# microsoft/DirectXTex

Hardware: AMD Instinct MI355X
Metric: Mtexels/s BC7 encode (4096^2 RGBA8, TEX_COMPRESS_DEFAULT) (higher is better)
Workload: dtype fp32 seed fit + i32 exact error sums (u8 texels in, 128-bit blocks out); 1 GPU; cfg2: 4096x4096 RGBA8 -> BC7_UNORM, TEX_COMPRESS_DEFAULT, one image per GPU, source and payload resident in HBM (dxtex_compress_device)

## Files before the change

### directxtex_amd/csrc/bc7_core.h

```cpp
#pragma once
#include <stdint.h>
#include <type_traits>

#if defined(DXTEX_HOST_DEBUG)
#define DXTEX_HD __host__ __device__ inline
#else
#define DXTEX_HD __device__ __forceinline__
#endif

namespace dxtex
{
namespace bc7
{
#if defined(DXTEX_HOST_DEBUG)
static bool g_hostFlatSkipEveryMode = true;
#endif
#if defined(DXTEX_COUNT_EVALS)
static long g_evalCount[8], g_evalTexels[8], g_macroCount[8], g_boundCount[8], g_pendCount[8], g_drainCount[8], g_pfTotal[8], g_pfPass[8], g_pfImprove[8], g_pfStepTotal[8][8], g_pfStepPass[8][8], g_tabWin[8], g_tabWinOut[8], g_tabWinOutPrev[8];
static int g_statTable = 0x7FFFFFFF, g_statTablePrev = 0x7FFFFFFF, g_statOther = 0;
static long g_rowCand[8], g_rowWin[8], g_rowTests[8][4], g_rowOut[8][4], g_rowDistN[8][6], g_rowDistOut[8][6], g_peelTests[8][4][3], g_peelOut[8][4][3];
#endif
template<int MODE> struct ModeInfo;
#define DXTEX_BC7_MODE(M, NS_, PARTBITS_, PB_, ROTBITS_, IMBITS_, IB_, IB2_, CP_, AP_, CPP_, APP_) \
    template<> struct ModeInfo<M> { enum : int { NS = NS_, PARTBITS = PARTBITS_, PB = PB_, ROTBITS = ROTBITS_, IMBITS = IMBITS_, \
// ... 1299 lines not shown
            ++g_pendCount[MODE];
#endif
        }
        exh_advance(s); --rem;
        const bool ended = rem == 0;
        if (n == 8 || ended)
        {
#if defined(DXTEX_COUNT_EVALS)
            if (n) ++g_drainCount[MODE];
#endif
            for (int j = n - 1; j >= 0; --j)
            {
                const uint32_t k = exh_key(exh_exact<MODE, IM, CHSET>(rg, vp, s.ch, s.aleb, s.o0, s.lo, queue[j], base), queue[j]);
                bestKey = k < bestKey ? k : bestKey;
            }
            n = 0;
        }
        if (ended)
        {
            exh_apply_key(s, bestKey);
            has = exh_next<MODE, IM, CHSET>(s, vp);
            skip_excluded();
            if (has) exh_peel<MODE, IM, CHSET>(rg, vp, s, base);
#if defined(DXTEX_ROW_STATS)
            row_stats(); peel_stats();
#endif
            if (has) { bestKey = exh_start_key(s); rem = exh_remaining(s); }
        }
    }
    optA = s.optA; optB = s.optB; optErr = s.optErr;
}

template<int MODE, int IM, class RG>
DXTEX_HD void optimize_one_lockstep(const RG& rg, int orgErr, uint32_t orgA, uint32_t orgB, uint32_t& optA, uint32_t& optB)
{
    optA = orgA; optB = orgB;
    int err = orgErr;
    if constexpr (PaletteBits<MODE, IM>::AB == 0)
    {
        lockstep_perturb_loop<MODE, IM, CH_ALL>(rg, optA, optB, err);
        lockstep_exhaustive_loop<MODE, IM, CH_ALL>(rg, optA, optB, err);
    }
    else
    {
        lockstep_perturb_loop<MODE, IM, CH_COLOR>(rg, optA, optB, err);
        lockstep_perturb_loop<MODE, IM, CH_ALPHA>(rg, optA, optB, err);
        lockstep_exhaustive_loop<MODE, IM, CH_COLOR>(rg, optA, optB, err);
        lockstep_exhaustive_loop<MODE, IM, CH_ALPHA>(rg, optA, optB, err);
    }
}

struct SubsetResult
{
    uint32_t orgA, orgB, optA, optB;
    uint64_t orgIdx1, orgIdx2, optIdx1, optIdx2;
    int orgErr, optErr;
};

template<int MODE, int IM, class RG>
DXTEX_HD void refine_pre(const RG& rg, uint32_t seedA, uint32_t seedB, uint32_t anchorPos, SubsetResult& out)
{
    const uint32_t qa = quantize_endpoint<MODE>(seedA), qb = quantize_endpoint<MODE>(seedB);
    fix_pbits<MODE>(qa, qb, out.orgA, out.orgB);
    out.orgErr = assign_indices<MODE, IM>(rg, out.orgA, out.orgB, anchorPos, out.orgIdx1, out.orgIdx2);
}

template<int MODE, int IM, class RG>
DXTEX_HD void refine_pre_err(const RG& rg, uint32_t seedA, uint32_t seedB, uint32_t anchorPos, SubsetResult& out)
{
    const uint32_t qa = quantize_endpoint<MODE>(seedA), qb = quantize_endpoint<MODE>(seedB);
    fix_pbits<MODE>(qa, qb, out.orgA, out.orgB);
    out.orgErr = assign_error<MODE, IM>(rg, out.orgA, out.orgB, anchorPos);
}

template<int MODE, int IM, class RG>
DXTEX_HD void refine_post(const RG& rg, uint32_t oa, uint32_t ob, uint32_t anchorPos, SubsetResult& out)
{
    fix_pbits<MODE>(oa, ob, out.optA, out.optB);
    out.optErr = assign_indices<MODE, IM>(rg, out.optA, out.optB, anchorPos, out.optIdx1, out.optIdx2);
}

template<int MODE, int IM, class RG>
DXTEX_HD void refine_subset(const RG& rg, uint32_t seedA, uint32_t seedB, uint32_t anchorPos, SubsetResult& out)
{
    refine_pre<MODE, IM>(rg, seedA, seedB, anchorPos, out);
    uint32_t oa, ob;
#if defined(DXTEX_BC7_USE_LOCKSTEP)
    optimize_one_lockstep<MODE, IM>(rg, out.orgErr, out.orgA, out.orgB, oa, ob);
#else
    optimize_one<MODE, IM>(rg, out.orgErr, out.orgA, out.orgB, oa, ob);
#endif
    refine_post<MODE, IM>(rg, oa, ob, anchorPos, out);
}

template<bool FULL, class F>
DXTEX_HD void for_masked(uint32_t mask16, F&& f)
{
    if constexpr (FULL)
    {
#pragma unroll
        for (int i = 0; i < 16; ++i) f(i);
    }
    else
    {
        for (uint32_t m = mask16 & 0xFFFFu; m; m &= m - 1u) f(int(__builtin_ctz(m)));
    }
}


template<bool RGBA, bool FULL = false, bool A1 = false>
DXTEX_HD bool fit_setup(const float* fpx, uint32_t mask16, float (&X)[4], float (&Y)[4])
{
// ... 456 lines not shown
```

### directxtex_amd/csrc/bc7_encode.hip

```cpp
#include "dxtex_kernels.h"
#include "bc67_tables.h"
#include "bc7_core.h"
#include "search_common.h"
#include <algorithm>
#include <cstdio>
#include <cstdlib>
#include <vector>

namespace dxtex
{
namespace
{
using namespace bc7;

struct Cand { uint32_t err; uint32_t ord; uint64_t lo, hi; };

enum : int { SLOT_M0 = 0, SLOT_M1, SLOT_M2, SLOT_M3, SLOT_M4A, SLOT_M4B, SLOT_M5, SLOT_M6, SLOT_M7, NUM_SLOTS };
enum : int { LIST_BYTES = 64 };

enum : int { PHASE_ALL = 0, PHASE_EARLY = 1, PHASE_LATE = 2 };

struct Bc7Args
{
    SegTable seg;
// ... 183 lines not shown
struct TaskRec { uint32_t A, B; int err; int orgErr; };

template<int MODE, int IM> struct TaskMap
{
    typedef ModeInfo<MODE> MI;
    enum : int { NS = MI::NS,
                 G = (NS == 1) ? 1 : (NS == 2) ? 2 : 4,
                 RANKS = (NS == 1) ? ((MODE == 6) ? 1 : 4) : ((MODE == 0) ? 4 : 16),
                 TPB = RANKS * G,
                 LIST = (MODE == 1) ? 0 : (MODE == 0) ? 33 : (MODE == 2) ? 40 : 16,
                 SLOT = (MODE == 0) ? SLOT_M0 : (MODE == 1) ? SLOT_M1 : (MODE == 2) ? SLOT_M2 : (MODE == 3) ? SLOT_M3 :
                        (MODE == 4) ? (IM ? SLOT_M4B : SLOT_M4A) : (MODE == 5) ? SLOT_M5 : (MODE == 6) ? SLOT_M6 : SLOT_M7 };
};

template<int MODE, int IM>
__device__ __forceinline__ uint32_t candidate_sub(uint32_t rank)
{
    return (TaskMap<MODE, IM>::NS == 1) ? ((MODE == 4) ? (rank * 2 + IM) * 16u : rank * 16u) : rank;
}
template<int MODE, int IM>
__device__ __forceinline__ uint32_t candidate_ord(uint32_t rank) { return uint32_t(MODE) * 128u + candidate_sub<MODE, IM>(rank); }

template<int MODE>
__device__ __forceinline__ bool phase_owns(const Bc7Args& a, uint32_t nb)
{
    if (a.phase == PHASE_ALL || (MODE != 4 && MODE != 5 && MODE != 6)) return true;
    const uint8_t* lst = a.lists + uint64_t(nb) * LIST_BYTES;
    const bool early = (MODE == 6) ? (lst[37] != 0 && a.flagged[0] >= a.early6Min) : (lst[32] != 0 && a.flagged[1] >= a.earlyAlphaMin);
    return early == (a.phase == PHASE_EARLY);
}

__device__ __forceinline__ bool lst_has_alpha(const Bc7Args& a, uint32_t nb) { return a.lists[uint64_t(nb) * LIST_BYTES + 32] != 0; }

template<int MODE, int IM>
__device__ __forceinline__ bool task_geometry(const Bc7Args& a, uint32_t nb, uint32_t r, uint32_t& shape, uint32_t& mask, uint32_t& anchor, uint32_t& rot)
{
    typedef TaskMap<MODE, IM> TM;
    shape = 0; mask = 0xFFFFu; anchor = 0; rot = 0;
    if (nb >= a.nblocks) return false;
    if (!phase_owns<MODE>(a, nb)) return false;
    const uint32_t rank = r / TM::G, region = r % TM::G;
    if (a.zeroOrd[nb] < candidate_ord<MODE, IM>(rank)) return false;
    if (TM::NS == 1) { rot = (MODE == 6) ? 0u : r; return true; }
    if (region >= uint32_t(TM::NS)) return false;
    const uint8_t* lst = a.lists + uint64_t(nb) * LIST_BYTES;
    if (MODE == 7 && lst[32] == 0) return false;
    shape = lst[TM::LIST + rank];
    if (TM::NS == 2)
    {
        const uint32_t m1 = kPart2Mask[shape];
        mask = region ? m1 : ((~m1) & 0xFFFFu);
        anchor = region ? uint32_t(kAnchor2[shape]) : 0u;
    }
    else
    {
        const uint32_t bits = kPart3Bits[shape];
        mask = 0;
#pragma unroll
        for (int i = 0; i < 16; ++i) if (((bits >> (2 * i)) & 3u) == region) mask |= 1u << i;
        anchor = (region == 0) ? 0u : (region == 1) ? uint32_t(kAnchor3[shape] & 15) : uint32_t(kAnchor3[shape] >> 4);
    }
    return true;
}

template<int MODE, int IM, bool ASSIGN = true>
__device__ __forceinline__ void task_org(const float* fpx, const uint32_t* pix, uint32_t mask, uint32_t anchor, uint32_t rot,
                                         SubsetResult& res, int& np, bool wantRegion, Region& rgOut, Block16& b16Out, const uint2* seed = nullptr)
{
    typedef TaskMap<MODE, IM> TM;
    if (TM::NS == 1)
    {
        block16_init(b16Out, pix, rot);
        uint32_t A, B;
        if (seed) { const uint2 sd = seed[(MODE == 6) ? 1 : 0]; A = sd.x; B = sd.y; }
        else if (MODE == 6) seed_endpoints<true>(fpx, 0xFFFFu, A, B);
// ... 24 lines not shown
    }
}

template<int BPW>
__device__ __forceinline__ void stage_packed(const Bc7Args& a, uint32_t nbFirst, int lane, uint32_t* sL)
{
    for (int t = lane; t < BPW * 16; t += 64)
    {
        const uint32_t nb = nbFirst + (uint32_t(t) >> 4);
        sL[t] = (nb < a.nblocks) ? a.px[uint64_t(nb) * 16 + (t & 15)] : 0u;
    }
    wave_lds_sync();
}

#if !defined(DXTEX_PP45_WGS)
#define DXTEX_PP45_WGS 1
#endif
template<int MODE, int IM>
__global__ void __launch_bounds__(256, (MODE == 4 || MODE == 5) ? DXTEX_PP45_WGS : 1) bc7_pre_kernel(Bc7Args a)
{
    typedef TaskMap<MODE, IM> TM;
    constexpr int BPW = (TM::TPB >= 64) ? 1 : 64 / TM::TPB;
    __shared__ uint32_t sL[4][BPW * 16];
    const int wave = threadIdx.x >> 6, lane = threadIdx.x & 63;
    const uint32_t nbFirst = (blockIdx.x * 4 + wave) * BPW;
    if (nbFirst >= a.nblocks) return;
    if (a.gate && *a.gate < a.gateMin) return;
    const uint32_t blk = uint32_t(lane) / TM::TPB, r = uint32_t(lane) % TM::TPB;
    const uint32_t nb = nbFirst + blk;
    uint32_t shape, mask, anchor, rot;
    const bool active = (blk < uint32_t(BPW)) && task_geometry<MODE, IM>(a, nb, r, shape, mask, anchor, rot);
    TaskRec rec; rec.A = 0; rec.B = 0; rec.err = 0; rec.orgErr = 0;
    uint32_t npLive = 0;
    if (!__any(active))
    {
        if (nb < a.nblocks && blk < uint32_t(BPW))
        {
            a.recs[uint64_t(nb) * TM::TPB + r] = rec;
            a.tinfo[uint64_t(nb) * TM::TPB + r] = 0;
        }
        return;
    }
    stage_packed<BPW>(a, nbFirst, lane, sL[wave]);
    int lb = 0;
    if (active)
    {
        SubsetResult res; int np; Region rg; Block16 b16;
        task_org<MODE, IM>(nullptr, &sL[wave][blk * 16], mask, anchor, rot, res, np, true, rg, b16,
                           (TM::NS == 2) ? a.seeds + uint64_t(nb) * 64 + (TM::LIST ? 32 : 0) + r
                                         : (TM::NS == 1) ? a.seeds1 + uint64_t(nb) * 2 : a.seeds3 + uint64_t(nb) * 192 + shape * 3 + (r % TM::G));
        rec.A = res.orgA; rec.B = res.orgB; rec.err = res.orgErr; rec.orgErr = res.orgErr;
        npLive = (res.orgErr != 0) ? uint32_t(np) : 0u;
        if (a.prune && npLive)
        {
            lb = subset_lower_bound(&sL[wave][blk * 16], mask, rot, (MODE >= 6) ? 4 : 3);
            if (MODE == 4 || MODE == 5)
            {
                if (rot != 0 || lst_has_alpha(a, nb))
                    lb += scalar_kmeans_lower_bound<(MODE == 4 && IM == 0) ? 8 : 4>(&sL[wave][blk * 16], rot);
            }
            if (MODE < 4)
            {
                const uint32_t* pix = &sL[wave][blk * 16];
#pragma unroll
                for (int i = 0; i < 16; ++i) if ((mask >> i) & 1u) { const int da = 255 - int(pix[i] >> 24); lb += da * da; }
            }
        }
    }
    if (a.prune)
    {
        int candOrg = active ? rec.err : 0, candLb = lb;
#pragma unroll
        for (int d = 1; d < TM::G; d <<= 1) { candOrg += __shfl_xor(candOrg, d); candLb += __shfl_xor(candLb, d); }
        int table = active ? candOrg : 0x7FFFFFFF;
#pragma unroll
        for (int d = TM::G; d < TM::TPB && d < 64; d <<= 1) table = min(table, __shfl_xor(table, d));
        if (nb < a.nblocks && blk < uint32_t(BPW)) table = min(table, a.bestErr[nb]);
        if (candLb > table) npLive = 0;
    }
    if (nb < a.nblocks && blk < uint32_t(BPW))
    {
        a.recs[uint64_t(nb) * TM::TPB + r] = rec;
        a.tinfo[uint64_t(nb) * TM::TPB + r] = (mask & 0xFFFFu) | (rot << 16) | (npLive << 24);
    }
}

template<int MODE, int IM>
__device__ __forceinline__ void search_pickup(const Bc7Args& a, uint2 task, uint32_t* slotCol, SlotRegion& rg)
{
    typedef TaskMap<MODE, IM> TM;
    const uint32_t nb = task.x / TM::TPB;
    const uint32_t mask = task.y & 0xFFFFu, rot = (task.y >> 16) & 3u;
    const uint4* px4 = reinterpret_cast<const uint4*>(a.px + uint64_t(nb) * 16);
    const uint4 q0 = px4[0], q1 = px4[1], q2 = px4[2], q3 = px4[3];
    const uint32_t px[16] = { q0.x, q0.y, q0.z, q0.w, q1.x, q1.y, q1.z, q1.w, q2.x, q2.y, q2.z, q2.w, q3.x, q3.y, q3.z, q3.w };
    int np = 0;
    if (TM::NS == 1)
    {
#pragma unroll
        for (int i = 0; i < 16; ++i) slotCol[i * kSlotStride] = rotate_pixel(px[i], rot);
        np = 16;
    }
    else
    {
#pragma unroll
        for (int i = 0; i < 16; ++i)
            if ((mask >> i) & 1u) { slotCol[np * kSlotStride] = px[i]; ++np; }
    }
    rg.base = slotCol; rg.np = np; rg.p2sum = 0;
}

__device__ __forceinline__ int lanes_below(unsigned long long mask)
{
    return int(__builtin_amdgcn_mbcnt_hi(uint32_t(mask >> 32), __builtin_amdgcn_mbcnt_lo(uint32_t(mask), 0u)));
}

// ... 671 lines not shown
                const int o = oStart + c / 11, i = st.lo + c % 11;
                const bool valid = c < 121 && o < st.oEnd && i < st.iEnd && i >= o;
                int e = 0x7FFFFFFF;
                if (valid)
                {
                    const int av = st.aleb ? o : i, bv = st.aleb ? i : o;
                    e = eval_var<MODE, IM, CHSET>(rg, vp, ch, unq1<C::PREC>(uint32_t(av)), unq1<C::PREC>(uint32_t(bv)), base);
                }
                const uint64_t key = valid ? ((uint64_t(uint32_t(e)) << 8) | uint32_t(c)) : ~0ull;
                bestKey = key < bestKey ? key : bestKey;
            }
#pragma unroll
            for (int d = 32; d > 0; d >>= 1)
            {
                const uint32_t lo = uint32_t(__shfl_xor(int(uint32_t(bestKey)), d)), hi = uint32_t(__shfl_xor(int(uint32_t(bestKey >> 32)), d));
                const uint64_t other = (uint64_t(hi) << 32) | lo;
                bestKey = other < bestKey ? other : bestKey;
            }
            if (bestKey != ~0ull)
            {
                const int e = int(uint32_t(bestKey >> 8)), c = int(bestKey & 0xFFu);
                if (e < st.best) { st.best = e; st.omin = oStart + c / 11; st.imin = st.lo + c % 11; }
            }
            st = exh_commit(st);
        }
        if (lane == 0)
        {
            TaskRec* r = a.recs + task.x;
            r->A = st.optA; r->B = st.optB; r->err = st.optErr;
        }
    }
}

template<int MODE, int IM>
__global__ void __launch_bounds__(256, (MODE == 4 || MODE == 5) ? DXTEX_PP45_WGS : 1) bc7_post_kernel(Bc7Args a)
{
    typedef TaskMap<MODE, IM> TM;
    constexpr int BPW = (TM::TPB >= 64) ? 1 : 64 / TM::TPB;
    __shared__ uint32_t sL[4][BPW * 16];
    const int wave = threadIdx.x >> 6, lane = threadIdx.x & 63;
    const uint32_t nbFirst = (blockIdx.x * 4 + wave) * BPW;
    if (nbFirst >= a.nblocks) return;
    if (a.gate && *a.gate < a.gateMin) return;
    const uint32_t blk = uint32_t(lane) / TM::TPB, r = uint32_t(lane) % TM::TPB;
    const uint32_t nb = nbFirst + blk;
    const uint32_t rank = r / TM::G, region = r % TM::G;
    uint32_t shape, mask, anchor, rot;
    const bool active = (blk < uint32_t(BPW)) && task_geometry<MODE, IM>(a, nb, r, shape, mask, anchor, rot);
    const bool mine = blk < uint32_t(BPW) && nb < a.nblocks && phase_owns<MODE>(a, nb);
    if (!__any(active))
    {
        if (mine && r == 0)
        {
            Cand c; c.err = 0xFFFFFFFFu; c.ord = 0xFFFFFFFFu; c.lo = 0; c.hi = 0;
            a.cands[uint64_t(nb) * NUM_SLOTS + TM::SLOT] = c;
        }
        return;
    }
    stage_packed<BPW>(a, nbFirst, lane, sL[wave]);

    SubsetResult res;
    res.orgErr = 0; res.optErr = 0; res.orgA = res.orgB = res.optA = res.optB = 0;
    res.orgIdx1 = res.orgIdx2 = res.optIdx1 = res.optIdx2 = 0;
    int np = 0; Region rg; Block16 b16;
    if (active)
    {
        task_org<MODE, IM, false>(nullptr, &sL[wave][blk * 16], mask, anchor, rot, res, np, true, rg, b16,
                                  (TM::NS == 2) ? a.seeds + uint64_t(nb) * 64 + (TM::LIST ? 32 : 0) + r
// ... 28 lines not shown
    uint64_t idx1 = myIdx1;
#pragma unroll
    for (int s = 1; s < TM::NS; ++s)
    {
        epA[s] = uint32_t(__shfl_down(int(myA), s));
        epB[s] = uint32_t(__shfl_down(int(myB), s));
        const uint64_t oi = uint64_t(uint32_t(__shfl_down(int(uint32_t(myIdx1)), s))) |
                            (uint64_t(uint32_t(__shfl_down(int(uint32_t(myIdx1 >> 32)), s))) << 32);
        idx1 |= oi;
    }

    if (blk < uint32_t(BPW) && nb < a.nblocks && region == 0)
    {
        if (active && key == best)
        {
            uint32_t anchors[3] = { 0, 0, 0 };
            if (TM::NS == 2) anchors[1] = kAnchor2[shape];
            if (TM::NS == 3) { anchors[1] = kAnchor3[shape] & 15; anchors[2] = kAnchor3[shape] >> 4; }
            Cand c;
            c.err = uint32_t(err);
            c.ord = uint32_t(MODE) * 128u + sub;
            emit_block<MODE>(shape, rot, IM, epA, epB, idx1, myIdx2, anchors, c.lo, c.hi);
            a.cands[uint64_t(nb) * NUM_SLOTS + TM::SLOT] = c;
            if (err == 0) atomicMin(&a.zeroOrd[nb], c.ord);
            atomicMin(&a.bestErr[nb], err);
        }
        else if (!active && rank == 0 && mine)
        {
            Cand c; c.err = 0xFFFFFFFFu; c.ord = 0xFFFFFFFFu; c.lo = 0; c.hi = 0;
            a.cands[uint64_t(nb) * NUM_SLOTS + TM::SLOT] = c;
        }
    }
}

template<bool RGBA>
__global__ void __launch_bounds__(256) bc7_block_seeds_kernel(Bc7Args a)
{
    const uint32_t nb = blockIdx.x * 256u + threadIdx.x;
    if (nb >= a.nblocks) return;
    const BcSeg& sg = seg_of(a.seg, nb);
    float f[64];
#pragma unroll
    for (int t = 0; t < 16; ++t) { uint32_t ldr; load_block_texel(sg.src, sg.nbw, sg.nb0 + (nb - sg.l0), uint32_t(t), &f[t * 4], ldr); }
    uint32_t A, B;
    seed_endpoints<RGBA, true>(f, 0xFFFFu, A, B);
    a.seeds1[uint64_t(nb) * 2 + (RGBA ? 1 : 0)] = make_uint2(A, B);
}

__global__ void __launch_bounds__(256) bc7_flag_count_kernel(Bc7Args a, uint32_t* out)
{
    uint32_t n = 0, m = 0;
    for (uint32_t nb = blockIdx.x * 256u + threadIdx.x; nb < a.nblocks; nb += gridDim.x * 256u)
    {
        uint8_t* lst = a.lists + uint64_t(nb) * LIST_BYTES;
        const bool hasAlpha = lst[32] != 0;
        bool first = hasAlpha;
        if (!first)
        {
            const uint4* px4 = reinterpret_cast<const uint4*>(a.px + uint64_t(nb) * 16);
            const uint4 q0 = px4[0], q1 = px4[1], q2 = px4[2], q3 = px4[3];
            const uint32_t px[16] = { q0.x, q0.y, q0.z, q0.w, q1.x, q1.y, q1.z, q1.w, q2.x, q2.y, q2.z, q2.w, q3.x, q3.y, q3.z, q3.w };
            const int ea = *reinterpret_cast<const int*>(lst + 56);
            first = int64_t(subset_lower_bound(px, 0xFFFFu, 0u, 4)) * 100 <= int64_t(ea) * a.early6Pct;
        }
        lst[37] = first ? 1 : 0;
        n += first ? 1u : 0u;
// ... 49 lines not shown
struct ScratchLayout
{
    size_t lists, cands, px, recs, order, tinfo, counters, zeroOrd, bestErr, seeds, seeds1, seeds3, flagcnt, auxRecs, auxOrder, auxTinfo, auxCounters, total;
    size_t auxTpb, auxSlices;
    explicit ScratchLayout(uint64_t nb, bool threeSubsets)
    {
        auto up = [](size_t v) { return (v + 255) & ~size_t(255); };
        const size_t tpb = threeSubsets ? kMaxTasksPerBlock : 32;
        const bool small = nb <= kSmallPassBlocks;
        auxTpb = small ? tpb : 4; auxSlices = small ? size_t(kSideStreams) : 2;
        size_t o = 0;
        lists = o; o = up(o + nb * LIST_BYTES);
        cands = o; o = up(o + nb * NUM_SLOTS * sizeof(Cand));
        px = o; o = up(o + nb * 64);
        recs = o; o = up(o + nb * tpb * sizeof(TaskRec));
        order = o; o = up(o + nb * tpb * sizeof(uint2));
        tinfo = o; o = up(o + nb * tpb * sizeof(uint32_t));
        counters = o; o = up(o + 64 * sizeof(uint32_t));
        zeroOrd = o; o = up(o + nb * sizeof(uint32_t));
        bestErr = o; o = up(o + nb * sizeof(int));
        seeds = o; o = up(o + nb * 64 * sizeof(uint2));
        seeds1 = o; o = up(o + nb * 2 * sizeof(uint2));
        seeds3 = o; o = up(o + (threeSubsets ? nb * 192 * sizeof(uint2) : 0));
        flagcnt = o; o = up(o + 256);
        auxRecs = o; o = up(o + auxSlices * nb * auxTpb * sizeof(TaskRec));
        auxOrder = o; o = up(o + auxSlices * nb * auxTpb * sizeof(uint2));
        auxTinfo = o; o = up(o + auxSlices * nb * auxTpb * sizeof(uint32_t));
        auxCounters = o; o = up(o + size_t(kSideStreams) * 64 * sizeof(uint32_t));
        total = o;
    }
};

template<int MODE, int IM>
void launch_mode(const Bc7Args& a0, hipStream_t stream, KernelMarks* marks, const char* const (&names)[7])
{
    typedef TaskMap<MODE, IM> TM;
    constexpr int BPW = (TM::TPB >= 64) ? 1 : 64 / TM::TPB;
    const uint32_t nb = a0.nblocks;
    const uint32_t ntasks = nb * uint32_t(TM::TPB);
    const uint32_t gridPP = (nb + 4 * BPW - 1) / (4 * BPW);
    constexpr bool kWhole = TM::NS == 1;
    constexpr uint32_t kExhMax = (MODE == 6) ? kWaveTaskMax : kWaveTaskMax45;
    static const bool noGroup = dev_env("DXTEX_BC7_NO_GROUP") != nullptr;
    const bool maybeShortP = kWhole && !noGroup && (MODE == 6 || ntasks <= 4u * kPerturbWaveMax);
    const bool maybeShortE = kWhole && !noGroup && (MODE == 6 || ntasks <= 4u * kExhMax);
    const uint32_t wavesP = std::min<uint32_t>(kSearchWaves, (ntasks + 1) / 2), wavesE = std::min<uint32_t>(kSearchWaves, ntasks);
    Bc7Args a = a0;
    a.gate = nullptr; a.gateMin = 0;
    if (a0.flagged && !(a0.flags & BCF_BC7_QUICK))
    {
        if (MODE == 7) { a.gate = a0.flagged + 1; a.gateMin = 1; }
        else if (a0.phase == PHASE_EARLY && (MODE == 4 || MODE == 5)) { a.gate = a0.flagged + 1; a.gateMin = std::max<uint32_t>(1u, a0.earlyAlphaMin); }
        else if (a0.phase == PHASE_EARLY && MODE == 6) { a.gate = a0.flagged; a.gateMin = std::max<uint32_t>(1u, a0.early6Min); }
    }
    a.perturbWaveMax = maybeShortP ? kPerturbWaveMax : 0u;
    a.exhWaveMax = maybeShortE ? kExhMax : 0u;
    if (marks) marks->mark(names[0]);
    hipLaunchKernelGGL((bc7_pre_kernel<MODE, IM>), dim3(gridPP), dim3(256), 0, stream, a);
    if (marks) marks->mark(names[1]);
    (void)hipMemsetAsync(a.counters, 0, 64 * sizeof(uint32_t), stream);
    const uint32_t binGroups = std::min<uint32_t>(kBinGroups, (ntasks + 255) / 256);
    hipLaunchKernelGGL(bc7_bin_count_kernel, dim3(binGroups), dim3(256), 0, stream, a.tinfo, ntasks, a.counters, a.gate, a.gateMin);
    hipLaunchKernelGGL(bc7_bin_scan_kernel, dim3(1), dim3(1), 0, stream, a.counters);
    hipLaunchKernelGGL(bc7_bin_scatter_kernel, dim3(binGroups), dim3(256), 0, stream, a.tinfo, ntasks, a.counters, a.order, a.gate, a.gateMin);
    if (marks) marks->mark(names[2]);
    const uint32_t waves = std::min<uint32_t>(kSearchWaves, (ntasks + 63) / 64);
    static const int tailBelow = dev_env("DXTEX_BC7_TAIL_BELOW") ? atoi(dev_env("DXTEX_BC7_TAIL_BELOW")) : 48;
// ... 5 lines not shown
        if constexpr (MODE == 1 || MODE == 6)
        {
            if (perturbPlain) hipLaunchKernelGGL((bc7_perturb_kernel<MODE, IM, CH_ALL>), dim3(waves), dim3(64), 0, stream, a, 0);
            else hipLaunchKernelGGL((bc7_perturb_filter_kernel<MODE, IM, CH_ALL>), dim3(waves), dim3(64), 0, stream, a, 0);
        }
        else
            hipLaunchKernelGGL((bc7_perturb_kernel<MODE, IM, CH_ALL>), dim3(waves), dim3(64), 0, stream, a, 0);
        if constexpr (kWhole) { if (maybeShortP) hipLaunchKernelGGL((bc7_perturb_wave_kernel<MODE, IM, CH_ALL>), dim3(wavesP), dim3(64), 0, stream, a); }
        if (marks) marks->mark(names[4]);
        if constexpr (kWhole) { if (maybeShortE) hipLaunchKernelGGL((bc7_exhaustive_wave_kernel<MODE, IM, CH_ALL>), dim3(wavesE), dim3(64), 0, stream, a); }
        hipLaunchKernelGGL((bc7_exhaustive_kernel<MODE, IM, CH_ALL>), dim3(waves), dim3(64), 0, stream, a, 1, tailBelow, rangeTests);
    }
    else
    {
        if constexpr (MODE == 4 && IM == 1 && DXTEX_PF_M4 != 0)
        {
            if (perturbPlain) hipLaunchKernelGGL((bc7_perturb_kernel<MODE, IM, CH_COLOR>), dim3(waves), dim3(64), 0, stream, a, 0);
            else hipLaunchKernelGGL((bc7_perturb_filter_kernel<MODE, IM, CH_COLOR>), dim3(waves), dim3(64), 0, stream, a, 0);
        }
        else
            hipLaunchKernelGGL((bc7_perturb_kernel<MODE, IM, CH_COLOR>), dim3(waves), dim3(64), 0, stream, a, 0);
        if (maybeShortP) hipLaunchKernelGGL((bc7_perturb_wave_kernel<MODE, IM, CH_COLOR>), dim3(wavesP), dim3(64), 0, stream, a);
        if (marks) marks->mark(names[3]);
        hipLaunchKernelGGL((bc7_perturb_kernel<MODE, IM, CH_ALPHA>), dim3(waves), dim3(64), 0, stream, a, 1);
        if (maybeShortP) hipLaunchKernelGGL((bc7_perturb_wave_kernel<MODE, IM, CH_ALPHA>), dim3(wavesP), dim3(64), 0, stream, a);
        if (marks) marks->mark(names[4]);
        if (maybeShortE) hipLaunchKernelGGL((bc7_exhaustive_wave_kernel<MODE, IM, CH_COLOR>), dim3(wavesE), dim3(64), 0, stream, a);
        hipLaunchKernelGGL((bc7_exhaustive_kernel<MODE, IM, CH_COLOR>), dim3(waves), dim3(64), 0, stream, a, 2, tailBelow, rangeTests);
        if (marks) marks->mark(names[5]);
        if (maybeShortE) hipLaunchKernelGGL((bc7_exhaustive_wave_kernel<MODE, IM, CH_ALPHA>), dim3(wavesE), dim3(64), 0, stream, a);
        hipLaunchKernelGGL((bc7_exhaustive_kernel<MODE, IM, CH_ALPHA>), dim3(waves), dim3(64), 0, stream, a, 3, tailBelow, rangeTests);
    }
    if (marks) marks->mark(names[6]);
    hipLaunchKernelGGL((bc7_post_kernel<MODE, IM>), dim3(gridPP), dim3(256), 0, stream, a);
#if defined(DXTEX_DEV)
    static const bool stats = dev_env("DXTEX_BC7_STATS") != nullptr;
    if (stats)
    {
        uint32_t c[40] = {};
        (void)hipStreamSynchronize(stream);
        (void)hipMemcpy(c, a.counters, sizeof(c), hipMemcpyDeviceToHost);
        std::fprintf(stderr, "bc7 stats %-22s phase %d: %9u task slots, %9u live; by size 16..1:", names[0], a.phase, ntasks, c[34]);
        for (int b = 16; b >= 1; --b) std::fprintf(stderr, " %u", c[b]);
        std::fprintf(stderr, "\n");
    }
#endif
}
}

#if defined(DXTEX_BC7_WAVETIMES)
namespace
{
void bc7_wavetimes_report()
{
    (void)hipDeviceSynchronize();
    static int call = 0;
    static const int wanted = dev_env("DXTEX_BC7_WT_CALL") ? atoi(dev_env("DXTEX_BC7_WT_CALL")) : 2;
    const bool print = call++ == wanted;
    static std::vector<unsigned long long> h(size_t(WT_KEYS) * 8192 * WT_FIELDS);
    static std::vector<unsigned int> hist(size_t(WT_KEYS) * 256);
    (void)hipMemcpyFromSymbol(h.data(), HIP_SYMBOL(g_wt), h.size() * 8);
    (void)hipMemcpyFromSymbol(hist.data(), HIP_SYMBOL(g_wtHist), hist.size() * 4);
    unsigned long long tAll = ~0ull;
    for (size_t i = 0; i < size_t(WT_KEYS) * 8192; ++i) if (h[i * WT_FIELDS + 2]) tAll = std::min(tAll, h[i * WT_FIELDS]);
    static const char* const kinds[3] = { "perturb", "perturb_filter", "exhaustive" };
    for (int key = 0; key < WT_KEYS; ++key)
    {
// ... 32 lines not shown
        }
        {
            const unsigned long long* e = w + idx[idx.size() / 2] * WT_FIELDS;
            std::fprintf(stderr, "    median wavefront %d: start %.0f drained %.0f end %.0f %% of span, rounds %llu, busy lanes / round %.1f, tasks %llu\n", idx[idx.size() / 2],
                         100.0 * double(e[0] - t0) / dur, 100.0 * double(e[1] - t0) / dur, 100.0 * double(e[2] - t0) / dur, e[3], e[3] ? double(e[4]) / e[3] : 0.0, e[5]);
        }
    }
    std::fill(h.begin(), h.end(), 0ull); std::fill(hist.begin(), hist.end(), 0u);
    (void)hipMemcpyToSymbol(HIP_SYMBOL(g_wt), h.data(), h.size() * 8);
    (void)hipMemcpyToSymbol(HIP_SYMBOL(g_wtHist), hist.data(), hist.size() * 4);
}
}
#endif

size_t bc7_scratch_bytes(uint64_t nblocks, uint32_t flags, size_t nimages)
{
    const bool three = (flags & BCF_USE_3SUBSETS) != 0;
    size_t need = ScratchLayout(nblocks < kMaxBlocksPerPass ? nblocks : kMaxBlocksPerPass, three).total;
    if (nblocks > kSmallPassBlocks) need = std::max(need, ScratchLayout(kSmallPassBlocks, three).total);
    return need + seg_table_bytes(nblocks, kMaxBlocksPerPass, nimages);
}

hipError_t launch_bc7_encode(const SrcView& src, uint8_t* dst, uint64_t dstRowPitch, uint32_t flags,
                             void* scratch, hipStream_t stream, KernelMarks* marks, const SideStreams* side)
{
    BcImage one; one.src = src; one.dst = dst; one.dstRowPitch = dstRowPitch;
    return launch_bc7_encode_many(&one, 1, flags, scratch, stream, marks, side);
}

hipError_t launch_bc7_encode_many(const BcImage* images, size_t count, uint32_t flags, void* scratch, hipStream_t stream, KernelMarks* marks,
                                  const SideStreams* side)
{
#define DXTEX_MARK(NAME) do { if (marks) marks->mark(NAME); } while (0)
#define DXTEX_MODE(MODE, IM, TAG) do { static const char* const n_[7] = { "bc7_pre_" TAG, "bc7_bin_" TAG, "bc7_perturb_" TAG, "bc7_perturb_alpha_" TAG, \
                                           "bc7_exhaustive_" TAG, "bc7_exhaustive_alpha_" TAG, "bc7_post_" TAG }; \
                                       launch_mode<MODE, IM>(a, stream, marks, n_); } while (0)
    std::vector<BcSeg> segs;
    std::vector<BcPass> passes;
    uint64_t perPass = 0;
    if (!build_passes(images, count, kMaxBlocksPerPass, segs, passes, &perPass)) return hipSuccess;
    const bool three = (flags & BCF_USE_3SUBSETS) != 0;
    const ScratchLayout L(perPass, three);
    uint8_t* base = static_cast<uint8_t*>(scratch);
    BcSeg* dSegs = reinterpret_cast<BcSeg*>(base + L.total);
    const hipError_t ce = upload_segments(dSegs, segs, passes, stream);
    if (ce != hipSuccess) return ce;
    const bool quick = (flags & BCF_BC7_QUICK) != 0;

    for (const BcPass& pass : passes)
    {
        Bc7Args a;
        set_pass(a.seg, dSegs, segs, pass);
        a.nblocks = pass.nblocks;
        a.flags = flags;
        a.perturbWaveMax = 0; a.exhWaveMax = 0;
        a.gate = nullptr; a.gateMin = 0;
        a.lists = base + L.lists;
        a.cands = reinterpret_cast<Cand*>(base + L.cands);
        a.px = reinterpret_cast<uint32_t*>(base + L.px);
        a.recs = reinterpret_cast<TaskRec*>(base + L.recs);
        a.order = reinterpret_cast<uint2*>(base + L.order);
        a.tinfo = reinterpret_cast<uint32_t*>(base + L.tinfo);
        a.counters = reinterpret_cast<uint32_t*>(base + L.counters);
        a.zeroOrd = reinterpret_cast<uint32_t*>(base + L.zeroOrd);
        a.bestErr = reinterpret_cast<int*>(base + L.bestErr);
        a.seeds = reinterpret_cast<uint2*>(base + L.seeds);
        a.seeds1 = reinterpret_cast<uint2*>(base + L.seeds1);
        a.seeds3 = reinterpret_cast<uint2*>(base + L.seeds3);
// ... 154 lines not shown
```

Before: 136.6 Mtexels/s.

## Split BC7 post into error-only selection and winner-only emit kernel

Result: no change. 137.7 Mtexels/s, median of 6 (+0.8%).

```diff
diff --git a/directxtex_amd/csrc/bc7_core.h b/directxtex_amd/csrc/bc7_core.h
--- a/directxtex_amd/csrc/bc7_core.h
+++ b/directxtex_amd/csrc/bc7_core.h
@@ -1355,7 +1355,7 @@
 }
 
 template<int MODE, int IM, class RG>
-DXTEX_HD void optimize_one_lockstep(const RG& rg, int orgErr, uint32_t orgA, uint32_t orgB, uint32_t& optA, uint32_t& optB)
+DXTEX_HD void optimize_one_lockstep(const RG& rg, int orgErr, uint32_t orgA, uint32_t orgB, uint32_t& optA, uint32_t& optB, int* errOut = nullptr)
 {
     optA = orgA; optB = orgB;
     int err = orgErr;
@@ -1371,6 +1371,7 @@
         lockstep_exhaustive_loop<MODE, IM, CH_COLOR>(rg, optA, optB, err);
         lockstep_exhaustive_loop<MODE, IM, CH_ALPHA>(rg, optA, optB, err);
     }
+    if (errOut) *errOut = err;
 }
 
 struct SubsetResult
@@ -1401,6 +1402,13 @@
 {
     fix_pbits<MODE>(oa, ob, out.optA, out.optB);
     out.optErr = assign_indices<MODE, IM>(rg, out.optA, out.optB, anchorPos, out.optIdx1, out.optIdx2);
+}
+
+template<int MODE, int IM, class RG>
+DXTEX_HD void refine_post_err(const RG& rg, uint32_t oa, uint32_t ob, uint32_t anchorPos, SubsetResult& out)
+{
+    fix_pbits<MODE>(oa, ob, out.optA, out.optB);
+    out.optErr = assign_error<MODE, IM>(rg, out.optA, out.optB, anchorPos);
 }
 
 template<int MODE, int IM, class RG>
diff --git a/directxtex_amd/csrc/bc7_encode.hip b/directxtex_amd/csrc/bc7_encode.hip
--- a/directxtex_amd/csrc/bc7_encode.hip
+++ b/directxtex_amd/csrc/bc7_encode.hip
@@ -239,15 +239,17 @@
 
 __device__ __forceinline__ bool lst_has_alpha(const Bc7Args& a, uint32_t nb) { return a.lists[uint64_t(nb) * LIST_BYTES + 32] != 0; }
 
-template<int MODE, int IM>
+constexpr uint32_t kTaskPruned = 1u << 23;
+
+template<int MODE, int IM, bool LIVE = true>
 __device__ __forceinline__ bool task_geometry(const Bc7Args& a, uint32_t nb, uint32_t r, uint32_t& shape, uint32_t& mask, uint32_t& anchor, uint32_t& rot)
 {
     typedef TaskMap<MODE, IM> TM;
     shape = 0; mask = 0xFFFFu; anchor = 0; rot = 0;
     if (nb >= a.nblocks) return false;
-    if (!phase_owns<MODE>(a, nb)) return false;
+    if (LIVE && !phase_owns<MODE>(a, nb)) return false;
     const uint32_t rank = r / TM::G, region = r % TM::G;
-    if (a.zeroOrd[nb] < candidate_ord<MODE, IM>(rank)) return false;
+    if (LIVE && a.zeroOrd[nb] < candidate_ord<MODE, IM>(rank)) return false;
     if (TM::NS == 1) { rot = (MODE == 6) ? 0u : r; return true; }
     if (region >= uint32_t(TM::NS)) return false;
     const uint8_t* lst = a.lists + uint64_t(nb) * LIST_BYTES;
@@ -338,6 +340,7 @@
     const bool active = (blk < uint32_t(BPW)) && task_geometry<MODE, IM>(a, nb, r, shape, mask, anchor, rot);
     TaskRec rec; rec.A = 0; rec.B = 0; rec.err = 0; rec.orgErr = 0;
     uint32_t npLive = 0;
+    uint32_t pruned = 0;
     if (!__any(active))
     {
         if (nb < a.nblocks && blk < uint32_t(BPW))
@@ -382,12 +385,12 @@
 #pragma unroll
         for (int d = TM::G; d < TM::TPB && d < 64; d <<= 1) table = min(table, __shfl_xor(table, d));
         if (nb < a.nblocks && blk < uint32_t(BPW)) table = min(table, a.bestErr[nb]);
-        if (candLb > table) npLive = 0;
+        if (candLb > table) { npLive = 0; pruned = kTaskPruned; }
     }
     if (nb < a.nblocks && blk < uint32_t(BPW))
     {
         a.recs[uint64_t(nb) * TM::TPB + r] = rec;
-        a.tinfo[uint64_t(nb) * TM::TPB + r] = (mask & 0xFFFFu) | (rot << 16) | (npLive << 24);
+        a.tinfo[uint64_t(nb) * TM::TPB + r] = (mask & 0xFFFFu) | (rot << 16) | pruned | (npLive << 24);
     }
 }
 
@@ -1125,8 +1128,157 @@
     }
 }
 
+constexpr uint32_t kParkedOpt = 1u << 31;
+
 template<int MODE, int IM>
 __global__ void __launch_bounds__(256, (MODE == 4 || MODE == 5) ? DXTEX_PP45_WGS : 1) bc7_post_kernel(Bc7Args a)
+{
+    typedef TaskMap<MODE, IM> TM;
+    constexpr int BPW = (TM::TPB >= 64) ? 1 : 64 / TM::TPB;
+    __shared__ uint32_t sL[4][BPW * 16];
+    const int wave = threadIdx.x >> 6, lane = threadIdx.x & 63;
+    const uint32_t nbFirst = (blockIdx.x * 4 + wave) * BPW;
+    if (nbFirst >= a.nblocks) return;
+    if (a.gate && *a.gate < a.gateMin) return;
+    const uint32_t blk = uint32_t(lane) / TM::TPB, r = uint32_t(lane) % TM::TPB;
+    const uint32_t nb = nbFirst + blk;
+    const uint32_t rank = r / TM::G, region = r % TM::G;
+    uint32_t shape, mask, anchor, rot;
+    bool active = (blk < uint32_t(BPW)) && task_geometry<MODE, IM>(a, nb, r, shape, mask, anchor, rot);
+    const bool mine = blk < uint32_t(BPW) && nb < a.nblocks && phase_owns<MODE>(a, nb);
+    if (active && (a.tinfo[uint64_t(nb) * TM::TPB + r] & kTaskPruned)) active = false;
+    if (!__any(active))
+    {
+        if (mine && r == 0)
+        {
+            Cand c; c.err = 0xFFFFFFFFu; c.ord = 0xFFFFFFFFu; c.lo = 0; c.hi = 0;
+            a.cands[uint64_t(nb) * NUM_SLOTS + TM::SLOT] = c;
+        }
+        return;
+    }
+    stage_packed<BPW>(a, nbFirst, lane, sL[wave]);
+
+    SubsetResult res;
+    res.orgErr = 0; res.optErr = 0; res.optA = res.optB = 0;
+    if (active)
+    {
+        const TaskRec rec = a.recs[uint64_t(nb) * TM::TPB + r];
+        res.orgErr = rec.orgErr;
+        if (TM::NS == 1)
+        {
+            Block16 b16; block16_init(b16, &sL[wave][blk * 16], rot);
+            refine_post_err<MODE, IM>(b16, rec.A, rec.B, 0u, res);
+        }
+        else
+        {
+            Region rg; region_init(rg, &sL[wave][blk * 16], mask);
+            refine_post_err<MODE, IM>(rg, rec.A, rec.B, anchor, res);
+        }
+    }
+    int orgTot = res.orgErr, optTot = res.optErr;
+#pragma unroll
+    for (int d = 1; d < TM::G; d <<= 1) { orgTot += __shfl_xor(orgTot, d); optTot += __shfl_xor(optTot, d); }
+    const bool useOpt = optTot < orgTot;
+    const int err = useOpt ? optTot : orgTot;
+    const uint32_t sub = candidate_sub<MODE, IM>(rank);
+    const uint32_t key = active ? ((uint32_t(err) << 7) | sub) : 0xFFFFFFFFu;
+    uint32_t best = key;
+#pragma unroll
+    for (int d = 1; d < TM::TPB && d < 64; d <<= 1) best = min(best, uint32_t(__shfl_xor(int(best), d)));
+    if (mine && region == 0)
+    {
+        if (active && key == best)
+        {
+            Cand c;
+            c.err = uint32_t(err);
+            c.ord = (uint32_t(MODE) * 128u + sub) | (useOpt ? kParkedOpt : 0u);
+            c.lo = 0; c.hi = 0;
+            a.cands[uint64_t(nb) * NUM_SLOTS + TM::SLOT] = c;
+            if (err == 0) atomicMin(&a.zeroOrd[nb], uint32_t(MODE) * 128u + sub);
+            atomicMin(&a.bestErr[nb], err);
+        }
+        else if (rank == 0 && best == 0xFFFFFFFFu)
+        {
+            Cand c; c.err = 0xFFFFFFFFu; c.ord = 0xFFFFFFFFu; c.lo = 0; c.hi = 0;
+            a.cands[uint64_t(nb) * NUM_SLOTS + TM::SLOT] = c;
+        }
+    }
+}
+
+template<int MODE, int IM>
+__global__ void __launch_bounds__(256) bc7_emit_kernel(Bc7Args a)
+{
+    typedef TaskMap<MODE, IM> TM;
+    constexpr int BPW = 64 / TM::G;
+    __shared__ uint32_t sL[4][(TM::NS == 1) ? 1 : BPW * 16];
+    const int wave = threadIdx.x >> 6, lane = threadIdx.x & 63;
+    const uint32_t nbFirst = (blockIdx.x * 4 + wave) * BPW;
+    if (nbFirst >= a.nblocks) return;
+    if (a.gate && *a.gate < a.gateMin) return;
+    const uint32_t blk = uint32_t(lane) / TM::G, region = uint32_t(lane) % TM::G;
+    const uint32_t nb = nbFirst + blk;
+    Cand c; c.err = 0xFFFFFFFFu; c.ord = 0; c.lo = 0; c.hi = 0;
+    if (nb < a.nblocks && phase_owns<MODE>(a, nb)) c = a.cands[uint64_t(nb) * NUM_SLOTS + TM::SLOT];
+    const bool won = c.err != 0xFFFFFFFFu;
+    if (!__any(won)) return;
+    if (TM::NS != 1) stage_packed<BPW>(a, nbFirst, lane, sL[wave]);
+
+    const bool useOpt = (c.ord & kParkedOpt) != 0;
+    const uint32_t ord = c.ord & ~kParkedOpt, sub = ord & 127u;
+    const uint32_t rank = (TM::NS != 1) ? sub : (MODE == 4) ? (sub >> 5) : (sub >> 4);
+    const uint32_t r = rank * TM::G + region;
+    uint32_t shape = 0, mask = 0xFFFFu, anchor = 0, rot = 0;
+    const bool active = won && task_geometry<MODE, IM, false>(a, nb, r, shape, mask, anchor, rot);
+    uint32_t myA = 0, myB = 0;
+    uint64_t myIdx1 = 0, myIdx2 = 0;
+    if (active)
+    {
+        SubsetResult res; int np; Region rg; Block16 b16;
+        uint32_t px[16];
+        if (TM::NS == 1)
+        {
+            const uint4* px4 = reinterpret_cast<const uint4*>(a.px + uint64_t(nb) * 16);
+            const uint4 q0 = px4[0], q1 = px4[1], q2 = px4[2], q3 = px4[3];
+            px[0] = q0.x; px[1] = q0.y; px[2] = q0.z; px[3] = q0.w; px[4] = q1.x; px[5] = q1.y; px[6] = q1.z; px[7] = q1.w;
+            px[8] = q2.x; px[9] = q2.y; px[10] = q2.z; px[11] = q2.w; px[12] = q3.x; px[13] = q3.y; px[14] = q3.z; px[15] = q3.w;
+        }
+        task_org<MODE, IM, false>(nullptr, (TM::NS == 1) ? px : &sL[wave][blk * 16], mask, anchor, rot, res, np, true, rg, b16,
+                                  (TM::NS == 2) ? a.seeds + uint64_t(nb) * 64 + (TM::LIST ? 32 : 0) + r
+                                                : (TM::NS == 1) ? a.seeds1 + uint64_t(nb) * 2 : a.seeds3 + uint64_t(nb) * 192 + shape * 3 + region);
+        myA = res.orgA; myB = res.orgB;
+        if (useOpt)
+        {
+            const TaskRec rec = a.recs[uint64_t(nb) * TM::TPB + r];
+            fix_pbits<MODE>(rec.A, rec.B, myA, myB);
+        }
+        if (TM::NS == 1) (void)assign_indices<MODE, IM>(b16, myA, myB, 0u, myIdx1, myIdx2);
+        else (void)assign_indices<MODE, IM>(rg, myA, myB, anchor, myIdx1, myIdx2);
+    }
+    uint32_t epA[3] = { myA, 0, 0 }, epB[3] = { myB, 0, 0 };
+    uint64_t idx1 = myIdx1;
+#pragma unroll
+    for (int s = 1; s < TM::NS; ++s)
+    {
+        epA[s] = uint32_t(__shfl_down(int(myA), s));
+        epB[s] = uint32_t(__shfl_down(int(myB), s));
+        const uint64_t oi = uint64_t(uint32_t(__shfl_down(int(uint32_t(myIdx1)), s))) |
+                            (uint64_t(uint32_t(__shfl_down(int(uint32_t(myIdx1 >> 32)), s))) << 32);
+        idx1 |= oi;
+    }
+    if (active && region == 0)
+    {
+        uint32_t anchors[3] = { 0, 0, 0 };
+        if (TM::NS == 2) anchors[1] = kAnchor2[shape];
+        if (TM::NS == 3) { anchors[1] = kAnchor3[shape] & 15; anchors[2] = kAnchor3[shape] >> 4; }
+        c.ord = ord;
+        emit_block<MODE>(shape, rot, IM, epA, epB, idx1, myIdx2, anchors, c.lo, c.hi);
+        a.cands[uint64_t(nb) * NUM_SLOTS + TM::SLOT] = c;
+    }
+}
+
+#if defined(DXTEX_DEV)
+template<int MODE, int IM>
+__global__ void __launch_bounds__(256, (MODE == 4 || MODE == 5) ? DXTEX_PP45_WGS : 1) bc7_post_full_kernel(Bc7Args a)
 {
     typedef TaskMap<MODE, IM> TM;
     constexpr int BPW = (TM::TPB >= 64) ? 1 : 64 / TM::TPB;
@@ -1221,6 +1373,7 @@
         }
     }
 }
+#endif
 
 template<bool RGBA>
 __global__ void __launch_bounds__(256) bc7_block_seeds_kernel(Bc7Args a)
@@ -1336,7 +1489,7 @@
 };
 
 template<int MODE, int IM>
-void launch_mode(const Bc7Args& a0, hipStream_t stream, KernelMarks* marks, const char* const (&names)[7])
+void launch_mode(const Bc7Args& a0, hipStream_t stream, KernelMarks* marks, const char* const (&names)[8])
 {
     typedef TaskMap<MODE, IM> TM;
     constexpr int BPW = (TM::TPB >= 64) ? 1 : 64 / TM::TPB;
@@ -1408,7 +1561,17 @@
         hipLaunchKernelGGL((bc7_exhaustive_kernel<MODE, IM, CH_ALPHA>), dim3(waves), dim3(64), 0, stream, a, 3, tailBelow, rangeTests);
     }
     if (marks) marks->mark(names[6]);
-    hipLaunchKernelGGL((bc7_post_kernel<MODE, IM>), dim3(gridPP), dim3(256), 0, stream, a);
+#if defined(DXTEX_DEV)
+    static const bool postFull = dev_env("DXTEX_BC7_POST_FULL") != nullptr;
+    if (postFull) hipLaunchKernelGGL((bc7_post_full_kernel<MODE, IM>), dim3(gridPP), dim3(256), 0, stream, a);
+    else
+#endif
+    {
+        hipLaunchKernelGGL((bc7_post_kernel<MODE, IM>), dim3(gridPP), dim3(256), 0, stream, a);
+        if (marks) marks->mark(names[7]);
+        constexpr uint32_t emitBlocks = 4 * (64 / TM::G);
+        hipLaunchKernelGGL((bc7_emit_kernel<MODE, IM>), dim3((nb + emitBlocks - 1) / emitBlocks), dim3(256), 0, stream, a);
+    }
 #if defined(DXTEX_DEV)
     static const bool stats = dev_env("DXTEX_BC7_STATS") != nullptr;
     if (stats)
@@ -1507,8 +1670,8 @@
                                   const SideStreams* side)
 {
 #define DXTEX_MARK(NAME) do { if (marks) marks->mark(NAME); } while (0)
-#define DXTEX_MODE(MODE, IM, TAG) do { static const char* const n_[7] = { "bc7_pre_" TAG, "bc7_bin_" TAG, "bc7_perturb_" TAG, "bc7_perturb_alpha_" TAG, \
-                                           "bc7_exhaustive_" TAG, "bc7_exhaustive_alpha_" TAG, "bc7_post_" TAG }; \
+#define DXTEX_MODE(MODE, IM, TAG) do { static const char* const n_[8] = { "bc7_pre_" TAG, "bc7_bin_" TAG, "bc7_perturb_" TAG, "bc7_perturb_alpha_" TAG, \
+                                           "bc7_exhaustive_" TAG, "bc7_exhaustive_alpha_" TAG, "bc7_post_" TAG, "bc7_emit_" TAG }; \
                                        launch_mode<MODE, IM>(a, stream, marks, n_); } while (0)
     std::vector<BcSeg> segs;
     std::vector<BcPass> passes;
```
